# pangenome/poasta

Hardware: AMD Instinct MI355X
Metric: Gcells/sec (aligned bases/sec in config), gap-affine POA alignment, 1k-node POA x 10k x 1 kbp queries per GPU (higher is better)
Workload: dtype u16

## Files before the change

### poasta_amd/csrc/poa_engine.hip

```cpp
#include <hip/hip_runtime.h>

#include <algorithm>
#include <array>
#include <chrono>
#include <cstdio>
#include <cstdlib>
#include <cstring>
#include <map>
#include <memory>
#include <new>
#include <mutex>
#include <string>
#include <vector>

#include "../../include/poasta_amd.h"
#include "poa_graph.hpp"
#include "poa_exact_kernel.hpp"
#include "poa_wsearch.hpp"
#include "poa_fsearch.hpp"

#include "poa_dense_plan.hpp"
#include "poa_kernels.hpp"
#include "poa_traceback_mf.hpp"
#include "poa_forward_packed.hpp"
// ... 146 lines not shown
    std::mutex bubble_mu;
};

struct poa_batch {
    const poa_graph* graph = nullptr;
    int device = 0;
    uint32_t n_queries = 0;
    uint64_t total_bases = 0, total_cells = 0, plane_bytes_total = 0;
    std::vector<uint64_t> h_qoff;
    std::vector<uint32_t> h_pitch;
    std::vector<uint64_t> h_scratch_off;
    struct Chunk { uint32_t first, count; };
    struct Plan {
        std::vector<Chunk> chunks;
        std::vector<uint64_t> off;
        uint32_t max_chunk = 0;
        DevBuf<uint64_t> d_off;
    };
    Plan plan[4];
    uint64_t plan_ws = 0;
    bool two_piece = false;
    bool plan16_same = true;
    int active_plan = 0;
    const Plan& cur() const { return plan[active_plan]; }
    uint64_t max_len = 0;
    bool narrow = false;
    bool compact = false;
    int cols_per_lane = 16;

    DevBuf<RowMeta> d_rows;
    DevBuf<uint32_t> d_pred_rows;
    DevBuf<uint32_t> d_row_depth, d_pred_k;
    DevBuf<uint32_t> d_dslot, d_pred_dslot;
    bool relative = false;
    bool dense_narrow = false, dense_compact = false, dense_relative = false, dense_derived_gaps = false;
    DevBuf<uint8_t> d_qseq;
    DevBuf<uint64_t> d_qoff, d_scratch_off, d_pair_off;
    DevBuf<uint32_t> d_pitch, d_carry, d_score, d_flags, d_npairs;
    PlaneWorkspace d_planes;
    DevBuf<uint2> d_scratch, d_pairs;
    DevBuf<uint32_t> d_succ_off, d_succ_rows, d_dist_min, d_dist_max, d_nbm_off, d_ex_status, d_exit_idx, d_ex_head, d_node_row, d_sp_to_end, d_ex_end;
    DevBuf<FlatGraph::NodeBubble> d_nbm;
    DevBuf<uint8_t> d_ex_sym;
    DevBuf<uint64_t> d_ex_reached, d_ex_rsum;
    DevBuf<ExQEntry> d_ex_pool;
    DevBuf<ExStackEntry> d_ex_stack;
    uint32_t ex_n_prio = 0, ex_pool_cap = 0, ex_stack_cap = 0, ex_wpn = 0, ex_swpn = 0;
    uint32_t ex_win = 64;
    uint32_t ex_skew = 0;
    DevBuf<uint32_t> d_ex_order;
    DevBuf<uint32_t> d_pipeline_error;
    DevBuf<unsigned long long> d_ex_prof;
    DevBuf<uint32_t> d_ex_counters;
    DevBuf<uint32_t> d_ex_logs;
    DevBuf<FlatGraph::RowRec> d_ex_rec;
    bool exact_ready = false;
    bool prof_on = false;
    uint32_t last_mode = 0;
    bool sweep = false;
    uint32_t sweep_slots = 1;
    uint64_t sweep_slotted = 0;
    uint64_t sweep_bytes_written = 0;
    bool ckpt = false;
    CheckpointPlan ckpt_plan;
    uint32_t ckpt_slots = 0;
    bool ckpt2 = false;
// ... 353 lines not shown
            HIP_TRY(hipGetLastError());
            fq.n_queries = 2 * n_narrow; bq.order = b->d_band_list_n.p + fp.first_query;
            bq.n_order = bn.count; bq.count_nf = b->d_band_count.p + 2 * n_chunks + ci;
            hipLaunchKernelGGL((poa_forward_band_kernel<false, true>), dim3((2 * n_narrow + 3) / 4), dim3(256), 0, stream, fq, bq);
            HIP_TRY(hipGetLastError());
            bq.n_order = nullptr; bq.count_nf = nullptr;
            b->narrow_ran += 2 * n_narrow; b->narrow_chunks = (uint32_t)ci + 1;
            b->narrow_how = R.band_narrow > 0 ? 2u : 1u;
        }
        if (n_pairs > n_narrow) {
            fq.n_queries = n_pairs - n_narrow; bq.order = b->d_band_order.p + ch.first + 2 * n_narrow;
            hipLaunchKernelGGL(poa_forward_band2_kernel<8>, dim3((n_pairs - n_narrow + 3) / 4), dim3(256), 0, stream, fq, bq);
        }
        if (n_single) {
            HIP_TRY(hipGetLastError());
            fq.n_queries = n_single; bq.order = b->d_band_order.p + ch.first + 2 * n_pairs;
            hipLaunchKernelGGL((poa_forward_band_kernel<false, true>), dim3((n_single + 3) / 4), dim3(256), 0, stream, fq, bq);
        }
        b->pair_paired += 2 * n_pairs; b->pair_single += n_single;
    } else {
        hipLaunchKernelGGL(poa_forward_band_kernel<false>, dim3(blocks), dim3(256), 0, stream, fp, bp);
        b->pair_single += ch.count;
    }
    HIP_TRY(hipGetLastError());
    hipLaunchKernelGGL(poa_forward_band_kernel<true>, dim3(blocks), dim3(256), 0, stream, fp, bp);
    uint32_t min_d = 0xFFFFFFFFu;
    for (uint32_t i = ch.first; i < ch.first + ch.count; ++i) min_d = std::min(min_d, std::min(b->h_band_d[b->h_band_cls[i]], R.band_cap));
    for (uint32_t k = 0; k < 2 * n_narrow; ++k) min_d = std::min(min_d, std::min(b->h_band_dn[b->h_band_cls[b->h_band_order[ch.first + k]]], R.band_cap));
    b->band_min_d = b->band_used ? std::min(b->band_min_d, min_d) : min_d;
    b->band_used = true; b->band_queries += ch.count; b->band_chunks = (uint32_t)ci + 1;
    return POA_OK;
}

void launch_traceback(const DenseRunPlan& R, const DenseChunkPlan& c, const TbParams& tp, hipStream_t stream) {
    const uint32_t lanes = c.v[5], per_block = 256 / lanes;
    const dim3 grid((c.v[7] + per_block - 1) / per_block), block(256);
    TbParams tpg = tp;
    tpg.spec_depth = c.v[6];
    if (c.lean_tb && lanes == 16) hipLaunchKernelGGL((poa_traceback_mf_kernel<16>), grid, block, 0, stream, tpg);
    else if (c.lean_tb && lanes == 32) hipLaunchKernelGGL((poa_traceback_mf_kernel<32>), grid, block, 0, stream, tpg);
    else if (c.lean_tb && lanes == 8) hipLaunchKernelGGL((poa_traceback_mf_kernel<8>), grid, block, 0, stream, tpg);
    else if (c.lean_tb) hipLaunchKernelGGL((poa_traceback_mf_kernel<64>), grid, block, 0, stream, tpg);
    else if (R.compact && lanes == 16) hipLaunchKernelGGL((poa_traceback_kernel<uint16_t, true, 16>), grid, block, 0, stream, tpg);
    else if (R.compact && lanes == 32) hipLaunchKernelGGL((poa_traceback_kernel<uint16_t, true, 32>), grid, block, 0, stream, tpg);
    else if (R.compact && lanes == 8) hipLaunchKernelGGL((poa_traceback_kernel<uint16_t, true, 8>), grid, block, 0, stream, tpg);
    else if (R.compact) hipLaunchKernelGGL((poa_traceback_kernel<uint16_t, true>), grid, block, 0, stream, tpg);
    else if (R.narrow) hipLaunchKernelGGL((poa_traceback_kernel<uint16_t, false>), grid, block, 0, stream, tp);
    else hipLaunchKernelGGL((poa_traceback_kernel<uint32_t, false>), grid, block, 0, stream, tp);
}

template <typename SearchParams>
void fill_search_params(SearchParams& sp, poa_batch* b, const ExactParams& ep, const TuneView& T) {
    sp.E = ep;
    sp.chunks = reinterpret_cast<ExU4*>(b->d_ex_pool.p);
    sp.chunk_cap = b->ex_pool_cap / BQ_CHUNK;
    if (const int* cv = T.ptr(POA_TUNE_WS_CHUNK_CAP)) { const int v = (*cv); if (v >= 1 && (uint32_t)v < sp.chunk_cap) sp.chunk_cap = (uint32_t)v; }
    sp.win = b->ex_win;
    sp.counters = b->d_ex_counters.p;
    sp.prof = T.ptr(POA_TUNE_WS_PROF) ? b->d_ex_prof.p : nullptr;
    sp.work_counter = nullptr; sp.order = nullptr;
}

uint32_t resident_blocks(poa_batch* b, const void* kfn, uint32_t wpb, uint32_t lds_bytes) {
    int per_cu = 1, cus = 256;
    (void)hipDeviceGetAttribute(&cus, hipDeviceAttributeMultiprocessorCount, b->device);
    if (hipOccupancyMaxActiveBlocksPerMultiprocessor(&per_cu, kfn, (int)(64 * wpb), lds_bytes) != hipSuccess || per_cu < 1) per_cu = 1;
    return (uint32_t)cus * (uint32_t)per_cu;
}

template <typename SearchParams>
int persistent_schedule(poa_batch* b, const poa_batch::Chunk& ch, uint32_t resident, hipStream_t stream, SearchParams& sp, uint32_t& n_blocks) {
    std::vector<uint32_t> sc(ch.count), ord(ch.count);
    HIP_TRY(hipMemcpyAsync(sc.data(), b->d_score.p + ch.first, (size_t)ch.count * 4, hipMemcpyDeviceToHost, stream));
    HIP_TRY(hipStreamSynchronize(stream));
    for (uint32_t i = 0; i < ch.count; ++i) ord[i] = i;
// ... 393 lines not shown
    if (ws == 0) {
        const uint64_t avail = free_b > fixed ? (uint64_t)((free_b - fixed) * 0.85) : 0;
        ws = std::min<uint64_t>(b->plane_bytes_total, avail);
    }
    if (sweep || ckpt) ws = std::min<uint64_t>(ws, b->plane_bytes_total);
    uint64_t biggest = 0;
    for (uint32_t i = 0; i < n_queries; ++i) biggest = std::max(biggest, q_plane_elems[i] * 4);
    if (ws < biggest) {
        if (workspace_bytes == 0 || workspace_bytes < biggest) {
            if (biggest + fixed > free_b)
                return fail(POA_ERR_OUT_OF_MEMORY, "score planes of the largest query do not fit in device memory");
            ws = biggest;
        }
    }
    auto make_plan = [&](poa_batch::Plan& pl, uint64_t elem_bytes, bool compact_size) {
        build_chunk_plan(pl, n_queries, ws, elem_bytes, [&](uint32_t i) {
            return compact_size ? compact_plane_elems(rows, b->h_pitch[i], fg.n_store_d) : q_plane_elems[i];
        });
    };
    b->plan_ws = ws;
    make_plan(b->plan[0], 4, false);
    b->plan16_same = sweep || b->plan[0].chunks.size() <= 1;
    if (!b->plan16_same) { make_plan(b->plan[1], 2, false); make_plan(b->plan[2], 2, !ckpt); }
    const uint32_t max_chunk_any = std::max(b->plan[0].max_chunk, std::max(b->plan[1].max_chunk, b->plan[2].max_chunk));
    b->cols_per_lane = 16;

    HIP_TRY(b->d_rows.alloc(fg.rows.size()));
    HIP_TRY(b->d_pred_rows.alloc(std::max<size_t>(fg.pred_rows.size(), 1)));
    HIP_TRY(b->d_pred_k.alloc(std::max<size_t>(fg.pred_k.size(), 1)));
    HIP_TRY(b->d_row_depth.alloc(std::max<size_t>(fg.row_depth.size(), 1)));
    const bool sweep_tables = sweep || ckpt;
    HIP_TRY(b->d_dslot.alloc(std::max<size_t>(sweep_tables ? g->sweep.slot.size() : fg.d_slot.size(), 1)));
    HIP_TRY(b->d_pred_dslot.alloc(std::max<size_t>(sweep_tables ? g->sweep.pred_slot.size() : fg.pred_dslot.size(), 1)));
    if (ckpt) {
        const CheckpointPlan& cp = b->ckpt_plan;
        HIP_TRY(b->d_ck_snap_off.alloc(cp.snap_off.size()));
        HIP_TRY(b->d_ck_snap_dst.alloc(std::max<size_t>(cp.snap_dst.size(), 1)));
        HIP_TRY(b->d_ck_pred_src.alloc(std::max<size_t>(cp.pred_src.size(), 1)));
        HIP_TRY(b->d_ck_boundary.alloc(cp.boundary.size()));
        HIP_TRY(hipMemcpy(b->d_ck_snap_off.p, cp.snap_off.data(), cp.snap_off.size() * 4, hipMemcpyHostToDevice));
        if (!cp.snap_dst.empty()) HIP_TRY(hipMemcpy(b->d_ck_snap_dst.p, cp.snap_dst.data(), cp.snap_dst.size() * 4, hipMemcpyHostToDevice));
        if (!cp.pred_src.empty()) HIP_TRY(hipMemcpy(b->d_ck_pred_src.p, cp.pred_src.data(), cp.pred_src.size() * 4, hipMemcpyHostToDevice));
        HIP_TRY(hipMemcpy(b->d_ck_boundary.p, cp.boundary.data(), cp.boundary.size() * 4, hipMemcpyHostToDevice));
    }
    HIP_TRY(b->d_qseq.alloc(std::max<uint64_t>(qoff[n_queries], 1)));
    HIP_TRY(b->d_qoff.alloc((size_t)n_queries + 1));
    HIP_TRY(b->d_pitch.alloc(std::max<uint32_t>(n_queries, 1)));
    for (int k = 0; k < (b->plan16_same ? 1 : 3); ++k) HIP_TRY(b->plan[k].d_off.alloc(std::max<uint32_t>(n_queries, 1)));
    HIP_TRY(b->d_scratch_off.alloc((size_t)n_queries + 1));
    HIP_TRY(b->d_pair_off.alloc((size_t)n_queries + 1));
    HIP_TRY(b->d_score.alloc(std::max<uint32_t>(n_queries, 1)));
    HIP_TRY(b->d_flags.alloc(std::max<uint32_t>(n_queries, 1)));
    HIP_TRY(b->d_npairs.alloc(std::max<uint32_t>(n_queries, 1)));
    HIP_TRY(b->d_scratch.alloc(std::max<uint64_t>(scratch_total, 1)));
    HIP_TRY(b->d_pairs.alloc(std::max<uint64_t>(scratch_total, 1)));
    HIP_TRY(b->d_carry.alloc(std::max<uint64_t>((sweep_tables ? (sweep_carry ? carry_words : 0ull) : 2ull) * max_chunk_any * rows, 1)));
    HIP_TRY(b->d_pipeline_error.alloc(1));
    HIP_TRY(hipMemset(b->d_pipeline_error.p, 0, 4));
    if (n_queries) {
        std::string werr;
        if (!b->d_planes.acquire(device, ws + 256, werr, sweep_tables)) return fail(POA_ERR_OUT_OF_MEMORY, "score-plane workspace: " + werr);
    }

    hipEvent_t e0, e1;
    HIP_TRY(hipEventCreate(&e0));
    HIP_TRY(hipEventCreate(&e1));
    HIP_TRY(hipEventRecord(e0, nullptr));
    HIP_TRY(hipMemcpy(b->d_rows.p, fg.rows.data(), fg.rows.size() * sizeof(RowMeta), hipMemcpyHostToDevice));
    if (!fg.pred_rows.empty())
        HIP_TRY(hipMemcpy(b->d_pred_rows.p, fg.pred_rows.data(), fg.pred_rows.size() * 4, hipMemcpyHostToDevice));
    if (!fg.pred_k.empty())
        HIP_TRY(hipMemcpy(b->d_pred_k.p, fg.pred_k.data(), fg.pred_k.size() * 4, hipMemcpyHostToDevice));
    if (!fg.row_depth.empty())
        HIP_TRY(hipMemcpy(b->d_row_depth.p, fg.row_depth.data(), fg.row_depth.size() * 4, hipMemcpyHostToDevice));
    const std::vector<uint32_t>& h_slot = sweep_tables ? g->sweep.slot : fg.d_slot;
    const std::vector<uint32_t>& h_pred_slot = sweep_tables ? g->sweep.pred_slot : fg.pred_dslot;
    if (!h_slot.empty())
        HIP_TRY(hipMemcpy(b->d_dslot.p, h_slot.data(), h_slot.size() * 4, hipMemcpyHostToDevice));
    if (!h_pred_slot.empty())
        HIP_TRY(hipMemcpy(b->d_pred_dslot.p, h_pred_slot.data(), h_pred_slot.size() * 4, hipMemcpyHostToDevice));
    if (sweep) HIP_TRY(hipMemset(b->d_pair_off.p, 0, ((size_t)n_queries + 1) * 8));
    if (qoff[n_queries]) HIP_TRY(hipMemcpy(b->d_qseq.p, qseq, qoff[n_queries], hipMemcpyHostToDevice));
    HIP_TRY(hipMemcpy(b->d_qoff.p, qoff, ((size_t)n_queries + 1) * 8, hipMemcpyHostToDevice));
    HIP_TRY(hipMemcpy(b->d_scratch_off.p, b->h_scratch_off.data(), ((size_t)n_queries + 1) * 8, hipMemcpyHostToDevice));
    if (n_queries) {
        HIP_TRY(hipMemcpy(b->d_pitch.p, b->h_pitch.data(), (size_t)n_queries * 4, hipMemcpyHostToDevice));
        for (int k = 0; k < (b->plan16_same ? 1 : 3); ++k)
            HIP_TRY(hipMemcpy(b->plan[k].d_off.p, b->plan[k].off.data(), (size_t)n_queries * 8, hipMemcpyHostToDevice));
    }
    HIP_TRY(hipEventRecord(e1, nullptr));
    HIP_TRY(hipEventSynchronize(e1));
    (void)hipEventElapsedTime(&b->ms_h2d, e0, e1);
    (void)hipEventDestroy(e0);
    (void)hipEventDestroy(e1);

    *out = b.release();
    return POA_OK;
}

static int prepare_exact(poa_batch* b, const poa_costs_t* costs, const poa_config_t* cfg) {
    const FlatGraph& fg = b->graph->g;
    std::string err;
    int rc;
    {
        std::lock_guard<std::mutex> lk(const_cast<poa_graph*>(b->graph)->bubble_mu);
        rc = build_bubble_index(const_cast<FlatGraph&>(fg), err);
    }
    if (rc != POA_OK) return fail(rc, err);
    const uint32_t n = fg.n;
    {
        uint32_t skew = 0;
        for (uint32_t r = 0; r < n; ++r) skew = std::max<uint32_t>(skew, fg.dist_max[r] - std::min(fg.dist_min[r], fg.dist_max[r]));
        b->ex_skew = skew;
// ... 225 lines not shown
        const DenseChunkPlan C = plan_dense_chunk(R, ch.count, max_pitch, T, compact_plane_elems(fg.n, max_pitch, fg.d_slot.empty() ? fg.n : fg.n_store_d));
        TbParams tp;
        tp.rows = b->d_rows.p; tp.pred_rows = b->d_pred_rows.p; tp.n_rows = fg.n;
        tp.start_row = fg.start_row; tp.end_row = fg.end_row;
        tp.first_query = ch.first; tp.n_queries = ch.count;
        tp.qseq = b->d_qseq.p; tp.qoff = b->d_qoff.p; tp.pitch = b->d_pitch.p; tp.plane_off = PL.d_off.p;
        tp.planes = b->d_planes.p; tp.scratch_off = b->d_scratch_off.p; tp.scratch = b->d_scratch.p;
        tp.score = b->d_score.p; tp.flags = b->d_flags.p; tp.n_pairs = b->d_npairs.p;
        tp.cost_x = costs->mismatch; tp.cost_o = costs->gap_open; tp.cost_e = costs->gap_extend;
        tp.spec_depth = R.spec_depth;
        tp.exact_pass = 0; tp.ex_status = nullptr; tp.ex_end = nullptr; tp.code_fmt = C.v[4];
        tp.row_depth = R.relative ? b->d_row_depth.p : nullptr;
        tp.d_slot = fg.d_slot.empty() ? nullptr : b->d_dslot.p; tp.pred_dslot = fg.d_slot.empty() ? nullptr : b->d_pred_dslot.p;
        FwdParams fp;
        fp.rows = b->d_rows.p; fp.pred_rows = b->d_pred_rows.p; fp.n_rows = fg.n;
        fp.first_query = ch.first; fp.n_queries = ch.count;
        fp.qseq = b->d_qseq.p; fp.qoff = b->d_qoff.p; fp.pitch = b->d_pitch.p; fp.plane_off = PL.d_off.p;
        fp.planes = b->d_planes.p; fp.strip_carry = b->d_carry.p;
        fp.cost_x = costs->mismatch; fp.cost_oe = (uint32_t)costs->gap_open + costs->gap_extend; fp.cost_e = costs->gap_extend;
        fp.cost_de = R.relative ? 0u : fp.cost_e;
        fp.cost_doe = R.relative ? (uint32_t)costs->gap_open : fp.cost_oe;
        fp.cost_ie = R.relative ? 2u * fp.cost_e : fp.cost_e;
        fp.cost_ioe = R.relative ? fp.cost_oe + fp.cost_e : fp.cost_oe;
        fp.pred_k = R.relative ? b->d_pred_k.p : nullptr;
        fp.d_slot = fg.d_slot.empty() ? nullptr : b->d_dslot.p; fp.pred_dslot = fg.d_slot.empty() ? nullptr : b->d_pred_dslot.p;
        fp.pipeline_error = b->d_pipeline_error.p;
        if (C.mf >= 0) b->dense_derived_gaps = C.mf == 3;
        if (C.band) { if (const int rc = launch_band(b, ci, R, fp, stream)) return rc; }
        else launch_forward(R, C, fp, tp, stream);
        HIP_TRY(hipGetLastError());
        if (const int rc = run.mark()) return rc;

        if (C.separate_tb) {
            launch_traceback(R, C, tp, stream);
            HIP_TRY(hipGetLastError());
            if (!C.lean_tb) b->tb_kernel = POA_TB_KERNEL_GENERIC;
            else if (b->tb_kernel == POA_TB_KERNEL_NONE) b->tb_kernel = POA_TB_KERNEL_LEAN;
            b->tb_lanes = C.v[5]; b->tb_depth = C.v[6]; b->tb_walks += C.v[7];
        }
        if (mode == POA_MODE_DENSE) b->launches.push_back(C);
        if (const int rc = run.mark()) return rc;

        if (mode != POA_MODE_DENSE) {
            if (const int rc = replay_chunk(b, ch, costs, cfg, T, mode == POA_MODE_HYBRID ? 1u : 0u, ends_free, tp, stream)) return rc;
        }
        if (const int rc = run.mark()) return rc;
    }
    return run.end_pairs();
}

int poa_batch_fetch(poa_batch_t* b, uint32_t* score, poa_aln_pair_t* pairs, uint64_t* pair_off, uint64_t pair_capacity,
                    uint32_t* flags, poa_stats_t* stats) {
    if (!b) return fail(POA_ERR_INVALID_ARG, "poa_batch_fetch: null batch");
    if (!b->ran) return fail(POA_ERR_INVALID_ARG, "poa_batch_fetch: poa_batch_run has not been called");
    HIP_TRY(hipSetDevice(b->device));
    HIP_TRY(hipStreamSynchronize(b->last_stream));
    {
        int prc = check_pipeline_error(b);
        if (prc != POA_OK) return prc;
    }
    const uint32_t n = b->n_queries;
    hipEvent_t e0, e1;
    HIP_TRY(hipEventCreate(&e0));
    HIP_TRY(hipEventCreate(&e1));
    HIP_TRY(hipEventRecord(e0, nullptr));
    std::vector<uint64_t> off_local;
    uint64_t* off = pair_off;
// ... 2032 lines not shown
```

### poasta_amd/csrc/poa_traceback_mf.hpp

```cpp
#pragma once
#include "poa_kernels.hpp"

namespace poa_amd {

struct MfCtx {
    const RowMeta* rows;
    const uint32_t* pred_rows;
    const uint16_t* M;
    const uint16_t* D;
    const uint32_t* d_slot;
    const uint32_t* pred_dslot;
    const uint8_t* q;
    uint32_t L, pitch, x, o, e;
    __device__ __forceinline__ uint32_t raw(uint32_t row, uint32_t j) const { return (uint32_t)M[row * pitch + j]; }
    __device__ __forceinline__ void cell(uint32_t row, uint32_t j, uint32_t& v, uint32_t& a, uint32_t& cf) const {
        const uint32_t r = raw(row, j);
        v = mf_value(r); a = (r >> 14) & 1u; cf = (r >> 15) & 1u;
    }
    __device__ __forceinline__ uint32_t m(uint32_t row, uint32_t j) const { return mf_value(raw(row, j)); }
    __device__ __forceinline__ uint32_t d_at(uint32_t slot, uint32_t j) const { return PlaneIO<uint16_t>::widen((uint32_t)D[slot * pitch + j]); }
    __device__ __forceinline__ uint32_t d_kept(uint32_t row, uint32_t j) const { return d_at(d_slot ? d_slot[row] : row, j); }
    __device__ __forceinline__ uint32_t pred(uint32_t k) const { return pred_rows[k]; }
    __device__ __forceinline__ uint32_t pred_d(uint32_t k, uint32_t j) const { return d_at(pred_dslot ? pred_dslot[k] : pred_rows[k], j); }
};

__device__ __forceinline__ void mf_cand(TbStep& f, uint32_t& n_cand, uint32_t row, uint32_t j, uint32_t st) {
    if (!f.found) { f.row = row; f.j = j; f.st = st; f.found = true; }
    n_cand++;
}
__device__ __forceinline__ uint32_t mf_sub(uint32_t a, uint32_t b, bool& panic) {
    const uint32_t r = a - b;
    if (r == INF) panic = true;
    return r;
}

template <bool END>
__device__ __forceinline__ TbStep mf_step_m(const MfCtx& c, const RowMeta& m, uint32_t row, uint32_t j, uint32_t raw, uint32_t up,
                                            uint32_t& n_cand, bool& panic) {
    TbStep f{0, 0, 0, false, 0, m.node};
    n_cand = 0;
    const uint32_t cs = mf_value(raw);
    f.cs = cs;
    if (cs == INF) return f;
    if (j > 0) {
        const bool moe = END || (uint32_t)m.sym == (uint32_t)c.q[j - 1];
        const uint32_t pj = END ? j : j - 1;
        const uint32_t target = (moe || m.pred_count == 0) ? cs : mf_sub(cs, c.x, panic);
        if (!END && (m.flags & ROW_CHAIN)) {
            if (up == target) mf_cand(f, n_cand, row - 1, pj, 0);
        } else {
            for (uint32_t k = 0; k < m.pred_count; ++k) {
                const uint32_t pr = c.pred_rows[m.pred_begin + k];
                if (c.m(pr, pj) == target) mf_cand(f, n_cand, pr, pj, 0);
            }
        }
    }
    if (raw & 0x8000u) mf_cand(f, n_cand, row, j, 1);
    if (raw & 0x4000u) mf_cand(f, n_cand, row, j, 2);
    return f;
}
__device__ __forceinline__ void mf_load_m(const MfCtx& c, uint32_t row, uint32_t j, uint32_t& raw, uint32_t& up) {
    const uint32_t off = row * c.pitch + j;
    raw = (uint32_t)c.M[off];
    up = (row > 0 && j > 0) ? mf_value((uint32_t)c.M[off - c.pitch - 1u]) : INF;
}

template <bool END>
__device__ __forceinline__ TbStep mf_step_d(const MfCtx& c, const RowMeta& m, uint32_t row, uint32_t j, uint32_t cs, uint32_t above,
                                            uint32_t& n_cand, bool& bad, bool& panic) {
    TbStep f{0, 0, 0, false, cs, m.node};
    n_cand = 0;
    if (cs == INF) return f;
    if (m.pred_count == 0) return f;
    const uint32_t t_open = mf_sub(mf_sub(cs, c.o, panic), c.e, panic), t_ext = mf_sub(cs, c.e, panic);
    const bool is_end = END || (m.flags & ROW_END) != 0;
    const bool real_open = !is_end && (j >= c.L || (uint32_t)m.sym != (uint32_t)c.q[j]);
    if (m.flags & ROW_CHAIN) {
        const uint32_t v = above;
        if (v == t_open) mf_cand(f, n_cand, row - 1, j, 0);
        else if (!real_open && v < t_open) bad = true;
        if (tbd_d_extends(c, row, j, cs)) mf_cand(f, n_cand, row - 1, j, 1);
    } else {
        for (uint32_t k = 0; k < m.pred_count; ++k) {
            const uint32_t pr = c.pred_rows[m.pred_begin + k];
            const uint32_t v = c.m(pr, j);
            if (v == t_open) mf_cand(f, n_cand, pr, j, 0);
            else if (!real_open && v < t_open) bad = true;
        }
        for (uint32_t k = 0; k < m.pred_count; ++k)
            if (c.pred_d(m.pred_begin + k, j) == t_ext) mf_cand(f, n_cand, c.pred_rows[m.pred_begin + k], j, 1);
    }
    return f;
}

__device__ __forceinline__ TbStep mf_step_i(const MfCtx& c, const RowMeta& m, uint32_t row, uint32_t j, uint32_t cs, uint32_t& n_cand,
                                            bool& bad, bool& panic) {
    TbStep f{0, 0, 0, false, cs, m.node};
    n_cand = 0;
    if (cs == INF) return f;
    if (j > 0) {
        const uint32_t t_open = mf_sub(mf_sub(cs, c.o, panic), c.e, panic), t_ext = mf_sub(cs, c.e, panic);
        const uint32_t pm = c.m(row, j - 1);
        if (pm == t_open) mf_cand(f, n_cand, row, j - 1, 0);
        else if (!tbd_open_i(c, m, j - 1) && pm < t_open) bad = true;
        if (tbd_i_extends(c, m, row, j, cs)) {
            const bool only = (n_cand == 0);
            mf_cand(f, n_cand, row, j - 1, 0);
            if (only && pm != t_ext) bad = true;
        }
    }
    return f;
}

template <int GW>
__device__ __forceinline__ void traceback_mf_walk(const TbParams& P, const uint32_t qi, const uint32_t lane) {
    const uint32_t gbase = (threadIdx.x & 63u) - lane;
    auto gballot = [&](bool pred) -> uint64_t {
        const uint64_t b = __ballot(pred);
        if (GW == 64) return b;
        const uint32_t w = (gbase & 32u) ? (uint32_t)(b >> 32) : (uint32_t)b;
        return (uint64_t)((w >> (gbase & 31u)) & (uint32_t)((1ull << (GW & 63)) - 1ull));
    };
    auto ones = [](uint64_t b) -> uint32_t { return (b == ~0ull) ? 64u : (uint32_t)__builtin_ctzll(~b); };
    auto bc = [&](uint32_t v, uint32_t src) { return (uint32_t)__shfl((int)v, (int)(gbase + src)); };

    const uint64_t qbeg = P.qoff[qi];
    MfCtx c;
    c.rows = P.rows; c.pred_rows = P.pred_rows;
    c.L = (uint32_t)(P.qoff[qi + 1] - qbeg);
    c.q = P.qseq + qbeg;
    c.pitch = P.pitch[qi];
    const uint64_t RP = (uint64_t)P.n_rows * c.pitch;
    c.M = reinterpret_cast<const uint16_t*>(P.planes) + P.plane_off[qi];
    c.D = c.M + RP + RP / 4;
    c.d_slot = P.d_slot; c.pred_dslot = P.pred_dslot;
    c.x = P.cost_x; c.o = P.cost_o; c.e = P.cost_e;
    const uint32_t L = c.L, start_row = P.start_row, end_row = P.end_row;

    uint2* out = P.scratch + P.scratch_off[qi];
    const uint32_t cap = (uint32_t)(P.scratch_off[qi + 1] - P.scratch_off[qi]);
    uint32_t cnt = 0;
    uint32_t flags = 0;
    uint32_t lflags = 0;
    auto emit_at = [&](uint32_t pos, uint32_t rpos, uint32_t qpos) {
        if (pos < cap) out[cap - 1 - pos] = make_uint2(rpos, qpos);
    };

    if (lane == 0) P.score[qi] = c.m(end_row, L);
    const uint32_t end_node = c.rows[end_row].node;

    bool done = false;
    uint32_t crow = 0, cj = 0, cst = 0;
    uint32_t gcs = INF;
    if (L == 0) done = true;
    if (!done && L == 1) {
        flags |= POA_FLAG_SHORT_QUERY;
        if (lane == 0) emit_at(0, end_node, 0);
        cnt = 1;
        done = true;
    }
    if (!done) {
        uint32_t f0 = 0, fr = 0, fj = 0, fs = 0, fallback = 0, fg = INF;
        if (lane == 0) {
            uint32_t nc; bool bad = false, pn = false;
            const RowMeta me = c.rows[end_row];
            TbStep cur = mf_step_m<true>(c, me, end_row, L, c.raw(end_row, L), INF, nc, pn);
            fg = cur.cs;
            if (cur.found && !pn && nc != 1) f0 |= POA_FLAG_AMBIGUOUS;
            if (!cur.found && !pn) {
                cur = mf_step_d<true>(c, me, end_row, L, c.d_kept(end_row, L), end_row > 0 ? c.m(end_row - 1, L) : INF, nc, bad, pn);
                fg = cur.cs;
                if (!pn) {
                    if (!cur.found) { f0 |= POA_FLAG_REF_PANIC; fallback = 1; }
                    else f0 |= POA_FLAG_AMBIGUOUS;
                    if (cur.found && cur.st == 1) fg = cur.cs - c.e;
                }
            }
            if (pn) { f0 |= POA_FLAG_REF_PANIC; fallback = 2; }
            fr = cur.row; fj = cur.j; fs = cur.st;
        }
        flags |= bc(f0, 0);
        const uint32_t fb = bc(fallback, 0);
        if (fb) {
            if (fb == 2) flags |= POA_FLAG_TRUNCATED;
            if (fb == 1 && L <= 3) {
                if (lane == 0) for (uint32_t i = 0; i < L; ++i) emit_at(i, end_node, L - 1 - i);
                cnt = L;
            }
            done = true;
        } else {
            crow = bc(fr, 0); cj = bc(fj, 0); cst = bc(fs, 0); gcs = bc(fg, 0);
        }
    }
    bool reached_start = done;
    uint32_t d_run = 0, i_run = 0;
    const uint32_t max_depth = P.spec_depth < (uint32_t)GW ? P.spec_depth : (uint32_t)GW;
    while (!done) {
        uint32_t depth = 1;
        if (cst == 2 && crow != start_row && max_depth > 1 && cj > 1) {
            uint32_t idepth = i_run < max_depth ? (i_run ? i_run : 1u) : max_depth;
            if (idepth < 2) idepth = 2;
            if (cj < idepth) idepth = cj;
            const bool iact = lane < idepth;
            const uint32_t jj = cj - lane;
            TbStep sI{0, 0, 0, false, 0, 0}, sM{0, 0, 0, false, 0, 0};
            uint32_t ncI = 0, ncM = 0;
            bool badI = false, pnI = false, pnM = false;
            RowMeta mi{};
            if (iact) {
                mi = c.rows[crow];
                uint32_t rawL, upL;
                mf_load_m(c, crow, jj - 1, rawL, upL);
                const uint32_t gcs_i = lane == 0 ? gcs : c.m(crow, jj);
                sI = mf_step_i(c, mi, crow, jj, gcs_i, ncI, badI, pnI);
                if (sI.found && !pnI) sM = mf_step_m<false>(c, mi, crow, sI.j, rawL, upL, ncM, pnM);
            }
            const bool cyc = iact && sI.found && !pnI && sI.j + 1 == jj && sM.found && !pnM && sM.st == 2 && sM.row == crow && sM.j == sI.j;
            const uint32_t ip = ones(gballot(cyc));
            if (ip > 0) {
                if (lane < ip) {
                    if (ncI != 1 || badI || ncM != 1) lflags |= POA_FLAG_AMBIGUOUS;
                    if (sI.j == 0 && (uint32_t)mi.sym == (uint32_t)c.q[0]) lflags |= POA_FLAG_START_QUIRK;
                    emit_at(cnt + lane, POA_NONE, jj - 1);
                }
                cnt += ip;
                cj -= ip;
                gcs = bc(sM.cs, ip - 1);
                i_run += ip;
                continue;
            }
            const uint32_t w0 = bc(((sI.found && !pnI) ? 1u : 0u) | ((ncI != 1 || badI) ? 2u : 0u), 0);
            if (w0 & 1u) {
                if (w0 & 2u) flags |= POA_FLAG_AMBIGUOUS;
                if (lane == 0) emit_at(cnt, POA_NONE, cj - 1);
                cnt += 1;
                const uint32_t n_row = crow, n_j = bc(sI.j, 0);
                if (n_j == 0 && (uint32_t)c.rows[n_row].sym == (uint32_t)c.q[0]) flags |= POA_FLAG_START_QUIRK;
                cj = n_j; cst = 0;
                i_run = 0;
                continue;
            }
        }
        if (cst != 2) i_run = 0;
        if (cst == 0) {
            depth = max_depth;
            if (crow + 1 < depth) depth = crow + 1;
            if (cj + 1 < depth) depth = cj + 1;
        } else if (cst == 1) {
            depth = d_run < max_depth ? (d_run ? d_run : 1u) : max_depth;
            if (crow + 1 < depth) depth = crow + 1;
        }
        if (cst != 1) d_run = 0;
        const bool active = lane < depth;
        const uint32_t my_row = crow - lane, my_j = (cst == 0) ? cj - lane : cj;
        TbStep bt{0, 0, 0, false, 0, 0};
        uint32_t nc = 0;
        bool bad = false, pn = false;
        if (active) {
            const RowMeta m = c.rows[my_row];
            if (cst == 0) {
                uint32_t raw, up;
                mf_load_m(c, my_row, my_j, raw, up);
                bt = mf_step_m<false>(c, m, my_row, my_j, raw, up, nc, pn);
            } else if (cst == 1) {
                const uint32_t above = my_row > 0 ? c.m(my_row - 1, my_j) : INF;
                bt = mf_step_d<false>(c, m, my_row, my_j, gcs - lane * c.e, above, nc, bad, pn);
            } else bt = mf_step_i(c, m, my_row, my_j, gcs, nc, bad, pn);
        }
        const bool amb = active && bt.found && (nc != 1 || bad);
        const bool quirk = active && bt.found && bt.st == 0 && bt.j == 0 && bt.row != start_row && cst != 1 &&
                           (uint32_t)c.rows[bt.row].sym == (uint32_t)c.q[0];
        const bool regular = active && bt.found && bt.row + 1 == my_row && bt.row != start_row &&
                             ((cst == 0 && bt.st == 0 && bt.j + 1 == my_j) || (cst == 1 && bt.st == 1 && bt.j == my_j));
        uint32_t p = ones(gballot(regular));
        bool dies = false;
        if (__ballot(active && pn)) {
            const uint64_t pnb = gballot(active && pn);
            const uint32_t first_pn = pnb ? (uint32_t)__builtin_ctzll(pnb) : 64u;
            dies = pnb != 0 && first_pn <= p;
            if (dies) p = first_pn;
        }
        if (lane < p) {
            if (amb) lflags |= POA_FLAG_AMBIGUOUS;
            if (quirk) lflags |= POA_FLAG_START_QUIRK;
            emit_at(cnt + lane, bt.node, cst == 0 ? my_j - 1 : POA_NONE);
        }
        cnt += p;
        if (dies) {
            flags |= POA_FLAG_REF_PANIC;
            break;
        }
        if (p == depth) {
            crow -= depth;
            if (cst == 0) cj -= depth;
            else { gcs -= depth * c.e; d_run += depth; }
            continue;
        }
        const uint32_t dw = bc((bt.found ? 1u : 0u) | (amb ? 2u : 0u) | (quirk ? 4u : 0u) | (bt.st << 3), p);
        const uint32_t d_row = bc(bt.row, p), d_j = bc(bt.j, p), d_cs = bc(bt.cs, p), d_node = bc(bt.node, p);
        const uint32_t d_st = dw >> 3;
        const uint32_t cur_j = (cst == 0) ? cj - p : cj, cur_st = cst;
        if (!(dw & 1u)) break;
        if (dw & 2u) flags |= POA_FLAG_AMBIGUOUS;
        if (cur_st == 0 && d_st != 0) {
            crow = d_row; cj = d_j; cst = d_st;
            gcs = d_cs;
            continue;
        }
        if (lane == 0) {
            if (cur_st == 0) emit_at(cnt, d_node, cur_j - 1);
            else if (cur_st == 2) emit_at(cnt, POA_NONE, cur_j - 1);
            else emit_at(cnt, d_node, POA_NONE);
        }
        cnt += 1;
        if (dw & 4u) flags |= POA_FLAG_START_QUIRK;
        if (d_row == start_row) { reached_start = true; break; }
        if (cur_st == 1 && d_st == 1) gcs = d_cs - c.e;
        if (cur_st == 1) d_run += p + 1;
        crow = d_row; cj = d_j; cst = d_st;
    }
    if (!reached_start) flags |= POA_FLAG_TRUNCATED;
    if (gballot((lflags & POA_FLAG_AMBIGUOUS) != 0)) flags |= POA_FLAG_AMBIGUOUS;
    if (gballot((lflags & POA_FLAG_START_QUIRK) != 0)) flags |= POA_FLAG_START_QUIRK;
    if (lane == 0) {
        P.flags[qi] = flags;
        P.n_pairs[qi] = cnt < cap ? cnt : cap;
    }
}

template <int GW>
__global__ __launch_bounds__(256) void poa_traceback_mf_kernel(TbParams P) {
    const uint32_t lane = threadIdx.x & (uint32_t)(GW - 1);
    const uint32_t wq = (blockIdx.x * blockDim.x + threadIdx.x) / (uint32_t)GW;
    if (wq >= P.n_queries) return;
    traceback_mf_walk<GW>(P, P.first_query + wq, lane);
}

}
```

Before: 2781.

## Pack per-row traceback metadata into 32-byte records and prefetch predecessor cells

Builds a packed 32-byte TbRow table per graph row on the host. Each record holds the node, symbol, flags, predecessor count, the first two predecessor rows, their D slots and the row's own D slot. The lean multi-lane traceback kernel now reads that one record instead of RowMeta, pred_rows, d_slot and pred_dslot separately. It also issues the M/D loads for up to two predecessors up front, before the candidate checks, to cut dependent gather chains. The cost is extra host setup and a device buffer. The table is only built when sweep/checkpoint tables are off, so the lean kernel would read a null table if it ever ran in those modes.

```diff
diff --git a/poasta_amd/csrc/poa_engine.hip b/poasta_amd/csrc/poa_engine.hip
--- a/poasta_amd/csrc/poa_engine.hip
+++ b/poasta_amd/csrc/poa_engine.hip
@@ -202,6 +202,7 @@
     DevBuf<uint32_t> d_pred_rows;
     DevBuf<uint32_t> d_row_depth, d_pred_k;
     DevBuf<uint32_t> d_dslot, d_pred_dslot;
+    DevBuf<TbRow> d_tb_rows;
     bool relative = false;
     bool dense_narrow = false, dense_compact = false, dense_relative = false, dense_derived_gaps = false;
     DevBuf<uint8_t> d_qseq;
@@ -621,15 +622,16 @@
     return POA_OK;
 }
 
-void launch_traceback(const DenseRunPlan& R, const DenseChunkPlan& c, const TbParams& tp, hipStream_t stream) {
+void launch_traceback(const DenseRunPlan& R, const DenseChunkPlan& c, const TbParams& tp, const TbRow* tb_rows, hipStream_t stream) {
     const uint32_t lanes = c.v[5], per_block = 256 / lanes;
     const dim3 grid((c.v[7] + per_block - 1) / per_block), block(256);
     TbParams tpg = tp;
     tpg.spec_depth = c.v[6];
-    if (c.lean_tb && lanes == 16) hipLaunchKernelGGL((poa_traceback_mf_kernel<16>), grid, block, 0, stream, tpg);
-    else if (c.lean_tb && lanes == 32) hipLaunchKernelGGL((poa_traceback_mf_kernel<32>), grid, block, 0, stream, tpg);
-    else if (c.lean_tb && lanes == 8) hipLaunchKernelGGL((poa_traceback_mf_kernel<8>), grid, block, 0, stream, tpg);
-    else if (c.lean_tb) hipLaunchKernelGGL((poa_traceback_mf_kernel<64>), grid, block, 0, stream, tpg);
+    const TbMfParams mf{tpg, tb_rows, tp.n_rows};
+    if (c.lean_tb && lanes == 16) hipLaunchKernelGGL((poa_traceback_mf_kernel<16>), grid, block, 0, stream, mf);
+    else if (c.lean_tb && lanes == 32) hipLaunchKernelGGL((poa_traceback_mf_kernel<32>), grid, block, 0, stream, mf);
+    else if (c.lean_tb && lanes == 8) hipLaunchKernelGGL((poa_traceback_mf_kernel<8>), grid, block, 0, stream, mf);
+    else if (c.lean_tb) hipLaunchKernelGGL((poa_traceback_mf_kernel<64>), grid, block, 0, stream, mf);
     else if (R.compact && lanes == 16) hipLaunchKernelGGL((poa_traceback_kernel<uint16_t, true, 16>), grid, block, 0, stream, tpg);
     else if (R.compact && lanes == 32) hipLaunchKernelGGL((poa_traceback_kernel<uint16_t, true, 32>), grid, block, 0, stream, tpg);
     else if (R.compact && lanes == 8) hipLaunchKernelGGL((poa_traceback_kernel<uint16_t, true, 8>), grid, block, 0, stream, tpg);
@@ -1089,6 +1091,11 @@
     const bool sweep_tables = sweep || ckpt;
     HIP_TRY(b->d_dslot.alloc(std::max<size_t>(sweep_tables ? g->sweep.slot.size() : fg.d_slot.size(), 1)));
     HIP_TRY(b->d_pred_dslot.alloc(std::max<size_t>(sweep_tables ? g->sweep.pred_slot.size() : fg.pred_dslot.size(), 1)));
+    std::vector<TbRow> h_tb_rows;
+    if (!sweep_tables) {
+        build_tb_rows(fg, h_tb_rows);
+        HIP_TRY(b->d_tb_rows.alloc(std::max<size_t>(h_tb_rows.size(), 1)));
+    }
     if (ckpt) {
         const CheckpointPlan& cp = b->ckpt_plan;
         HIP_TRY(b->d_ck_snap_off.alloc(cp.snap_off.size()));
@@ -1136,6 +1143,8 @@
         HIP_TRY(hipMemcpy(b->d_dslot.p, h_slot.data(), h_slot.size() * 4, hipMemcpyHostToDevice));
     if (!h_pred_slot.empty())
         HIP_TRY(hipMemcpy(b->d_pred_dslot.p, h_pred_slot.data(), h_pred_slot.size() * 4, hipMemcpyHostToDevice));
+    if (!h_tb_rows.empty())
+        HIP_TRY(hipMemcpy(b->d_tb_rows.p, h_tb_rows.data(), h_tb_rows.size() * sizeof(TbRow), hipMemcpyHostToDevice));
     if (sweep) HIP_TRY(hipMemset(b->d_pair_off.p, 0, ((size_t)n_queries + 1) * 8));
     if (qoff[n_queries]) HIP_TRY(hipMemcpy(b->d_qseq.p, qseq, qoff[n_queries], hipMemcpyHostToDevice));
     HIP_TRY(hipMemcpy(b->d_qoff.p, qoff, ((size_t)n_queries + 1) * 8, hipMemcpyHostToDevice));
@@ -1427,7 +1436,7 @@
         if (const int rc = run.mark()) return rc;
 
         if (C.separate_tb) {
-            launch_traceback(R, C, tp, stream);
+            launch_traceback(R, C, tp, b->d_tb_rows.p, stream);
             HIP_TRY(hipGetLastError());
             if (!C.lean_tb) b->tb_kernel = POA_TB_KERNEL_GENERIC;
             else if (b->tb_kernel == POA_TB_KERNEL_NONE) b->tb_kernel = POA_TB_KERNEL_LEAN;
diff --git a/poasta_amd/csrc/poa_tb_rows.cpp b/poasta_amd/csrc/poa_tb_rows.cpp
--- /dev/null
+++ b/poasta_amd/csrc/poa_tb_rows.cpp
@@ -0,0 +1,28 @@
+#include "poa_tb_rows.hpp"
+
+#include <algorithm>
+
+namespace poa_amd {
+
+void build_tb_rows(const FlatGraph& g, std::vector<TbRow>& out) {
+    const bool by_row = g.d_slot.empty();
+    out.assign(g.rows.size(), TbRow{});
+    for (size_t r = 0; r < g.rows.size(); ++r) {
+        const RowMeta& m = g.rows[r];
+        TbRow& t = out[r];
+        t.node = m.node;
+        t.pred_begin = m.pred_begin;
+        t.sym = m.sym; t.child_sym = m.child_sym; t.flags = m.flags;
+        t.npred = (uint8_t)std::min<uint32_t>(m.pred_count, TBR_NPRED_MORE);
+        uint32_t* p[2] = {&t.p0, &t.p1};
+        uint32_t* ds[2] = {&t.ds0, &t.ds1};
+        for (uint32_t k = 0; k < 2; ++k) {
+            const bool has = k < m.pred_count;
+            *p[k] = has ? g.pred_rows[m.pred_begin + k] : TBR_NONE;
+            *ds[k] = !has ? TBR_NONE : by_row ? *p[k] : g.pred_dslot[m.pred_begin + k];
+        }
+        t.dslot = by_row ? (uint32_t)r : g.d_slot[r];
+    }
+}
+
+}
diff --git a/poasta_amd/csrc/poa_tb_rows.hpp b/poasta_amd/csrc/poa_tb_rows.hpp
--- /dev/null
+++ b/poasta_amd/csrc/poa_tb_rows.hpp
@@ -0,0 +1,25 @@
+#pragma once
+#include <cstdint>
+#include <vector>
+
+#include "poa_graph.hpp"
+
+namespace poa_amd {
+
+constexpr uint32_t TBR_NONE = 0xFFFFFFFFu;
+constexpr uint8_t TBR_NPRED_MORE = 255;
+
+struct alignas(32) TbRow {
+    uint32_t node;
+    uint32_t pred_begin;
+    uint8_t sym, child_sym, flags;
+    uint8_t npred;
+    uint32_t p0, p1;
+    uint32_t ds0, ds1;
+    uint32_t dslot;
+};
+static_assert(sizeof(TbRow) == 32, "TbRow layout");
+
+void build_tb_rows(const FlatGraph& g, std::vector<TbRow>& out);
+
+}
diff --git a/poasta_amd/csrc/poa_traceback_mf.hpp b/poasta_amd/csrc/poa_traceback_mf.hpp
--- a/poasta_amd/csrc/poa_traceback_mf.hpp
+++ b/poasta_amd/csrc/poa_traceback_mf.hpp
@@ -1,14 +1,32 @@
 #pragma once
 #include "poa_kernels.hpp"
+#include "poa_tb_rows.hpp"
 
 namespace poa_amd {
 
+struct TbMfParams {
+    TbParams tp;
+    const TbRow* tb_rows;
+    uint32_t n_tb_rows;
+};
+
+struct MfRows {
+    const TbRow* t;
+    const RowMeta* meta;
+    __device__ __forceinline__ uint32_t npred(const TbRow& r, uint32_t row) const {
+        return r.npred != TBR_NPRED_MORE ? (uint32_t)r.npred : meta[row].pred_count;
+    }
+    __device__ __forceinline__ RowMeta of(const TbRow& r, uint32_t row) const {
+        return RowMeta{r.node, r.pred_begin, npred(r, row), r.sym, r.child_sym, r.flags, 0};
+    }
+    __device__ __forceinline__ RowMeta operator[](uint32_t row) const { return of(t[row], row); }
+};
+
 struct MfCtx {
-    const RowMeta* rows;
+    MfRows rows;
     const uint32_t* pred_rows;
     const uint16_t* M;
     const uint16_t* D;
-    const uint32_t* d_slot;
     const uint32_t* pred_dslot;
     const uint8_t* q;
     uint32_t L, pitch, x, o, e;
@@ -19,7 +37,7 @@
     }
     __device__ __forceinline__ uint32_t m(uint32_t row, uint32_t j) const { return mf_value(raw(row, j)); }
     __device__ __forceinline__ uint32_t d_at(uint32_t slot, uint32_t j) const { return PlaneIO<uint16_t>::widen((uint32_t)D[slot * pitch + j]); }
-    __device__ __forceinline__ uint32_t d_kept(uint32_t row, uint32_t j) const { return d_at(d_slot ? d_slot[row] : row, j); }
+    __device__ __forceinline__ uint32_t d_kept(uint32_t row, uint32_t j) const { return d_at(rows.t[row].dslot, j); }
     __device__ __forceinline__ uint32_t pred(uint32_t k) const { return pred_rows[k]; }
     __device__ __forceinline__ uint32_t pred_d(uint32_t k, uint32_t j) const { return d_at(pred_dslot ? pred_dslot[k] : pred_rows[k], j); }
 };
@@ -34,61 +52,99 @@
     return r;
 }
 
+struct MfLoadM {
+    uint32_t raw, qc, v0, v1;
+    __device__ __forceinline__ void req(const MfCtx& c, uint32_t row, uint32_t j) {
+        const uint32_t off = row * c.pitch + j;
+        raw = (uint32_t)c.M[off];
+        v0 = (row > 0 && j > 0) ? (uint32_t)c.M[off - c.pitch - 1u] : 0xFFFFu;
+        qc = j > 0 ? (uint32_t)c.q[j - 1] : 0u;
+        v1 = INF;
+    }
+    __device__ __forceinline__ void preds(const MfCtx& c, const TbRow& r, uint32_t j) {
+        uint32_t a = v0, b = 0xFFFFu;
+        if (!(r.flags & ROW_CHAIN) && j > 0) {
+            a = 0xFFFFu;
+            if (r.npred > 0) a = c.raw(r.p0, j - 1);
+            if (r.npred > 1) b = c.raw(r.p1, j - 1);
+        }
+        v0 = mf_value(a); v1 = mf_value(b);
+    }
+};
+
 template <bool END>
-__device__ __forceinline__ TbStep mf_step_m(const MfCtx& c, const RowMeta& m, uint32_t row, uint32_t j, uint32_t raw, uint32_t up,
+__device__ __forceinline__ TbStep mf_step_m(const MfCtx& c, const TbRow& r, uint32_t row, uint32_t j, const MfLoadM& ld,
                                             uint32_t& n_cand, bool& panic) {
-    TbStep f{0, 0, 0, false, 0, m.node};
+    TbStep f{0, 0, 0, false, 0, r.node};
     n_cand = 0;
-    const uint32_t cs = mf_value(raw);
+    const uint32_t raw = ld.raw, cs = mf_value(raw);
     f.cs = cs;
     if (cs == INF) return f;
     if (j > 0) {
-        const bool moe = END || (uint32_t)m.sym == (uint32_t)c.q[j - 1];
+        const uint32_t npred = c.rows.npred(r, row);
+        const bool moe = END || (uint32_t)r.sym == ld.qc;
         const uint32_t pj = END ? j : j - 1;
-        const uint32_t target = (moe || m.pred_count == 0) ? cs : mf_sub(cs, c.x, panic);
-        if (!END && (m.flags & ROW_CHAIN)) {
-            if (up == target) mf_cand(f, n_cand, row - 1, pj, 0);
-        } else {
-            for (uint32_t k = 0; k < m.pred_count; ++k) {
-                const uint32_t pr = c.pred_rows[m.pred_begin + k];
-                if (c.m(pr, pj) == target) mf_cand(f, n_cand, pr, pj, 0);
-            }
+        const uint32_t target = (moe || npred == 0) ? cs : mf_sub(cs, c.x, panic);
+        if (npred > 0 && ld.v0 == target) mf_cand(f, n_cand, r.p0, pj, 0);
+        if (npred > 1 && ld.v1 == target) mf_cand(f, n_cand, r.p1, pj, 0);
+        for (uint32_t k = 2; k < npred; ++k) {
+            const uint32_t pr = c.pred_rows[r.pred_begin + k];
+            if (c.m(pr, pj) == target) mf_cand(f, n_cand, pr, pj, 0);
         }
     }
     if (raw & 0x8000u) mf_cand(f, n_cand, row, j, 1);
     if (raw & 0x4000u) mf_cand(f, n_cand, row, j, 2);
     return f;
 }
-__device__ __forceinline__ void mf_load_m(const MfCtx& c, uint32_t row, uint32_t j, uint32_t& raw, uint32_t& up) {
-    const uint32_t off = row * c.pitch + j;
-    raw = (uint32_t)c.M[off];
-    up = (row > 0 && j > 0) ? mf_value((uint32_t)c.M[off - c.pitch - 1u]) : INF;
-}
+
+struct MfLoadD {
+    uint32_t qc, v0, v1, d0, d1;
+    __device__ __forceinline__ void req(const MfCtx& c, uint32_t row, uint32_t j) {
+        v0 = row > 0 ? (uint32_t)c.M[(row - 1u) * c.pitch + j] : 0xFFFFu;
+        qc = j < c.L ? (uint32_t)c.q[j] : 0u;
+        v1 = d0 = d1 = INF;
+    }
+    __device__ __forceinline__ void preds(const MfCtx& c, const TbRow& r, uint32_t j) {
+        uint32_t a = v0, b = 0xFFFFu, da = 0xFFFFu, db = 0xFFFFu;
+        if (!(r.flags & ROW_CHAIN)) {
+            a = 0xFFFFu;
+            if (r.npred > 0) { a = c.raw(r.p0, j); da = (uint32_t)c.D[r.ds0 * c.pitch + j]; }
+            if (r.npred > 1) { b = c.raw(r.p1, j); db = (uint32_t)c.D[r.ds1 * c.pitch + j]; }
+        }
+        v0 = mf_value(a); v1 = mf_value(b);
+        d0 = PlaneIO<uint16_t>::widen(da); d1 = PlaneIO<uint16_t>::widen(db);
+    }
+};
 
 template <bool END>
-__device__ __forceinline__ TbStep mf_step_d(const MfCtx& c, const RowMeta& m, uint32_t row, uint32_t j, uint32_t cs, uint32_t above,
+__device__ __forceinline__ TbStep mf_step_d(const MfCtx& c, const TbRow& r, uint32_t row, uint32_t j, uint32_t cs, const MfLoadD& ld,
                                             uint32_t& n_cand, bool& bad, bool& panic) {
-    TbStep f{0, 0, 0, false, cs, m.node};
+    TbStep f{0, 0, 0, false, cs, r.node};
     n_cand = 0;
     if (cs == INF) return f;
-    if (m.pred_count == 0) return f;
+    const uint32_t npred = c.rows.npred(r, row);
+    if (npred == 0) return f;
     const uint32_t t_open = mf_sub(mf_sub(cs, c.o, panic), c.e, panic), t_ext = mf_sub(cs, c.e, panic);
-    const bool is_end = END || (m.flags & ROW_END) != 0;
-    const bool real_open = !is_end && (j >= c.L || (uint32_t)m.sym != (uint32_t)c.q[j]);
-    if (m.flags & ROW_CHAIN) {
-        const uint32_t v = above;
-        if (v == t_open) mf_cand(f, n_cand, row - 1, j, 0);
+    const bool is_end = END || (r.flags & ROW_END) != 0;
+    const bool real_open = !is_end && (j >= c.L || (uint32_t)r.sym != ld.qc);
+    auto open = [&](uint32_t v, uint32_t pr) {
+        if (v == t_open) mf_cand(f, n_cand, pr, j, 0);
         else if (!real_open && v < t_open) bad = true;
+    };
+    if (r.flags & ROW_CHAIN) {
+        open(ld.v0, row - 1);
         if (tbd_d_extends(c, row, j, cs)) mf_cand(f, n_cand, row - 1, j, 1);
     } else {
-        for (uint32_t k = 0; k < m.pred_count; ++k) {
-            const uint32_t pr = c.pred_rows[m.pred_begin + k];
-            const uint32_t v = c.m(pr, j);
-            if (v == t_open) mf_cand(f, n_cand, pr, j, 0);
-            else if (!real_open && v < t_open) bad = true;
-        }
-        for (uint32_t k = 0; k < m.pred_count; ++k)
-            if (c.pred_d(m.pred_begin + k, j) == t_ext) mf_cand(f, n_cand, c.pred_rows[m.pred_begin + k], j, 1);
+        open(ld.v0, r.p0);
+        if (npred > 1) open(ld.v1, r.p1);
+        for (uint32_t k = 2; k < npred; ++k) {
+            const uint32_t pr = c.pred_rows[r.pred_begin + k];
+            open(c.m(pr, j), pr);
+        }
+        if (ld.d0 == t_ext) mf_cand(f, n_cand, r.p0, j, 1);
+        if (npred > 1 && ld.d1 == t_ext) mf_cand(f, n_cand, r.p1, j, 1);
+        for (uint32_t k = 2; k < npred; ++k)
+            if (c.pred_d(r.pred_begin + k, j) == t_ext) mf_cand(f, n_cand, c.pred_rows[r.pred_begin + k], j, 1);
     }
     return f;
 }
@@ -113,7 +169,8 @@
 }
 
 template <int GW>
-__device__ __forceinline__ void traceback_mf_walk(const TbParams& P, const uint32_t qi, const uint32_t lane) {
+__device__ __forceinline__ void traceback_mf_walk(const TbMfParams& PM, const uint32_t qi, const uint32_t lane) {
+    const TbParams& P = PM.tp;
     const uint32_t gbase = (threadIdx.x & 63u) - lane;
     auto gballot = [&](bool pred) -> uint64_t {
         const uint64_t b = __ballot(pred);
@@ -126,14 +183,14 @@
 
     const uint64_t qbeg = P.qoff[qi];
     MfCtx c;
-    c.rows = P.rows; c.pred_rows = P.pred_rows;
+    c.rows.t = PM.tb_rows; c.rows.meta = P.rows; c.pred_rows = P.pred_rows;
     c.L = (uint32_t)(P.qoff[qi + 1] - qbeg);
     c.q = P.qseq + qbeg;
     c.pitch = P.pitch[qi];
     const uint64_t RP = (uint64_t)P.n_rows * c.pitch;
     c.M = reinterpret_cast<const uint16_t*>(P.planes) + P.plane_off[qi];
     c.D = c.M + RP + RP / 4;
-    c.d_slot = P.d_slot; c.pred_dslot = P.pred_dslot;
+    c.pred_dslot = P.pred_dslot;
     c.x = P.cost_x; c.o = P.cost_o; c.e = P.cost_e;
     const uint32_t L = c.L, start_row = P.start_row, end_row = P.end_row;
 
@@ -147,7 +204,7 @@
     };
 
     if (lane == 0) P.score[qi] = c.m(end_row, L);
-    const uint32_t end_node = c.rows[end_row].node;
+    const uint32_t end_node = c.rows.t[end_row].node;
 
     bool done = false;
     uint32_t crow = 0, cj = 0, cst = 0;
@@ -163,12 +220,18 @@
         uint32_t f0 = 0, fr = 0, fj = 0, fs = 0, fallback = 0, fg = INF;
         if (lane == 0) {
             uint32_t nc; bool bad = false, pn = false;
-            const RowMeta me = c.rows[end_row];
-            TbStep cur = mf_step_m<true>(c, me, end_row, L, c.raw(end_row, L), INF, nc, pn);
+            const TbRow me = c.rows.t[end_row];
+            MfLoadM lm;
+            lm.raw = c.raw(end_row, L); lm.qc = 0;
+            lm.v0 = me.npred > 0 ? c.m(me.p0, L) : INF; lm.v1 = me.npred > 1 ? c.m(me.p1, L) : INF;
+            TbStep cur = mf_step_m<true>(c, me, end_row, L, lm, nc, pn);
             fg = cur.cs;
             if (cur.found && !pn && nc != 1) f0 |= POA_FLAG_AMBIGUOUS;
             if (!cur.found && !pn) {
-                cur = mf_step_d<true>(c, me, end_row, L, c.d_kept(end_row, L), end_row > 0 ? c.m(end_row - 1, L) : INF, nc, bad, pn);
+                MfLoadD ldd;
+                ldd.req(c, end_row, L);
+                ldd.preds(c, me, L);
+                cur = mf_step_d<true>(c, me, end_row, L, c.d_kept(end_row, L), ldd, nc, bad, pn);
                 fg = cur.cs;
                 if (!pn) {
                     if (!cur.found) { f0 |= POA_FLAG_REF_PANIC; fallback = 1; }
@@ -206,21 +269,22 @@
             TbStep sI{0, 0, 0, false, 0, 0}, sM{0, 0, 0, false, 0, 0};
             uint32_t ncI = 0, ncM = 0;
             bool badI = false, pnI = false, pnM = false;
-            RowMeta mi{};
+            TbRow ri{};
             if (iact) {
-                mi = c.rows[crow];
-                uint32_t rawL, upL;
-                mf_load_m(c, crow, jj - 1, rawL, upL);
+                ri = c.rows.t[crow];
+                MfLoadM lm;
+                lm.req(c, crow, jj - 1);
                 const uint32_t gcs_i = lane == 0 ? gcs : c.m(crow, jj);
-                sI = mf_step_i(c, mi, crow, jj, gcs_i, ncI, badI, pnI);
-                if (sI.found && !pnI) sM = mf_step_m<false>(c, mi, crow, sI.j, rawL, upL, ncM, pnM);
+                lm.preds(c, ri, jj - 1);
+                sI = mf_step_i(c, c.rows.of(ri, crow), crow, jj, gcs_i, ncI, badI, pnI);
+                if (sI.found && !pnI) sM = mf_step_m<false>(c, ri, crow, sI.j, lm, ncM, pnM);
             }
             const bool cyc = iact && sI.found && !pnI && sI.j + 1 == jj && sM.found && !pnM && sM.st == 2 && sM.row == crow && sM.j == sI.j;
             const uint32_t ip = ones(gballot(cyc));
             if (ip > 0) {
                 if (lane < ip) {
                     if (ncI != 1 || badI || ncM != 1) lflags |= POA_FLAG_AMBIGUOUS;
-                    if (sI.j == 0 && (uint32_t)mi.sym == (uint32_t)c.q[0]) lflags |= POA_FLAG_START_QUIRK;
+                    if (sI.j == 0 && (uint32_t)ri.sym == (uint32_t)c.q[0]) lflags |= POA_FLAG_START_QUIRK;
                     emit_at(cnt + lane, POA_NONE, jj - 1);
                 }
                 cnt += ip;
@@ -235,7 +299,7 @@
                 if (lane == 0) emit_at(cnt, POA_NONE, cj - 1);
                 cnt += 1;
                 const uint32_t n_row = crow, n_j = bc(sI.j, 0);
-                if (n_j == 0 && (uint32_t)c.rows[n_row].sym == (uint32_t)c.q[0]) flags |= POA_FLAG_START_QUIRK;
+                if (n_j == 0 && (uint32_t)c.rows.t[n_row].sym == (uint32_t)c.q[0]) flags |= POA_FLAG_START_QUIRK;
                 cj = n_j; cst = 0;
                 i_run = 0;
                 continue;
@@ -257,19 +321,22 @@
         uint32_t nc = 0;
         bool bad = false, pn = false;
         if (active) {
-            const RowMeta m = c.rows[my_row];
+            const TbRow r = c.rows.t[my_row];
             if (cst == 0) {
-                uint32_t raw, up;
-                mf_load_m(c, my_row, my_j, raw, up);
-                bt = mf_step_m<false>(c, m, my_row, my_j, raw, up, nc, pn);
+                MfLoadM lm;
+                lm.req(c, my_row, my_j);
+                lm.preds(c, r, my_j);
+                bt = mf_step_m<false>(c, r, my_row, my_j, lm, nc, pn);
             } else if (cst == 1) {
-                const uint32_t above = my_row > 0 ? c.m(my_row - 1, my_j) : INF;
-                bt = mf_step_d<false>(c, m, my_row, my_j, gcs - lane * c.e, above, nc, bad, pn);
-            } else bt = mf_step_i(c, m, my_row, my_j, gcs, nc, bad, pn);
+                MfLoadD ldd;
+                ldd.req(c, my_row, my_j);
+                ldd.preds(c, r, my_j);
+                bt = mf_step_d<false>(c, r, my_row, my_j, gcs - lane * c.e, ldd, nc, bad, pn);
+            } else bt = mf_step_i(c, c.rows.of(r, my_row), my_row, my_j, gcs, nc, bad, pn);
         }
         const bool amb = active && bt.found && (nc != 1 || bad);
         const bool quirk = active && bt.found && bt.st == 0 && bt.j == 0 && bt.row != start_row && cst != 1 &&
-                           (uint32_t)c.rows[bt.row].sym == (uint32_t)c.q[0];
+                           (uint32_t)c.rows.t[bt.row].sym == (uint32_t)c.q[0];
         const bool regular = active && bt.found && bt.row + 1 == my_row && bt.row != start_row &&
                              ((cst == 0 && bt.st == 0 && bt.j + 1 == my_j) || (cst == 1 && bt.st == 1 && bt.j == my_j));
         uint32_t p = ones(gballot(regular));
@@ -329,11 +396,12 @@
 }
 
 template <int GW>
-__global__ __launch_bounds__(256) void poa_traceback_mf_kernel(TbParams P) {
+__global__ __launch_bounds__(256) void poa_traceback_mf_kernel(TbMfParams PM) {
+    const TbParams& P = PM.tp;
     const uint32_t lane = threadIdx.x & (uint32_t)(GW - 1);
     const uint32_t wq = (blockIdx.x * blockDim.x + threadIdx.x) / (uint32_t)GW;
     if (wq >= P.n_queries) return;
-    traceback_mf_walk<GW>(P, P.first_query + wq, lane);
-}
-
-}
+    traceback_mf_walk<GW>(PM, P.first_query + wq, lane);
+}
+
+}
```

After: 2402. 0.864x the previous value.
